# sunilsarolkarcds/ISL-SignLanguage-Translation

Hardware: AMD Instinct MI355X
Metric: frames/sec body_25 368×656 fwd+NMS+PAF at 1/8 MI355X; conv MFMA util % (higher is better)
Workload: dtype fp32 (split-fp16 x3 MFMA, fp32 accumulate)

## Files before the change

### isl-signlanguage-translation_amd/csrc/wino_f16.hip

```cpp
#include <algorithm>
#include <cstdlib>
#include <type_traits>

#include "internal.h"

namespace isl {
namespace {

typedef _Float16 f16x8 __attribute__((ext_vector_type(8)));
typedef _Float16 f16x2 __attribute__((ext_vector_type(2)));
typedef float f32x2 __attribute__((ext_vector_type(2)));
typedef float f32x4 __attribute__((ext_vector_type(4)));
typedef float f32x16 __attribute__((ext_vector_type(16)));
typedef unsigned u32x4 __attribute__((ext_vector_type(4)));

struct W2Args {
  const float* in;
  float* out;
  const f16x8* upk;
  const float* bias;
  const float* slope;
  int* range_flag;
  long long in_fs, in_chs, out_fs, out_chs;
  float wscale_inv;
  int in_pad, out_pad, H, W, TH, TW, pairs, cin_chunks, co_blocks, bpf, act, nblocks;
};

constexpr int RS = 34;
constexpr int QS = 6 * 2 * RS;
constexpr int HS = 13 * 64;
constexpr int BUF = 32 * 64;

__device__ __forceinline__ void split_dw(const f32x4& v, unsigned& h01, unsigned& h23, unsigned& l01, unsigned& l23) {
  asm("v_cvt_pk_f16_f32 %0, %1, %2" : "=v"(h01) : "v"(v.x), "v"(v.y));
  asm("v_cvt_pk_f16_f32 %0, %1, %2" : "=v"(h23) : "v"(v.z), "v"(v.w));
  asm("v_fma_mixlo_f16 %0, %1, -1.0, %2 op_sel_hi:[1,0,0]" : "=v"(l01) : "v"(h01), "v"(v.x));
  asm("v_fma_mixhi_f16 %0, %1, -1.0, %2 op_sel:[1,0,0] op_sel_hi:[1,0,0]" : "+v"(l01) : "v"(h01), "v"(v.y));
  asm("v_fma_mixlo_f16 %0, %1, -1.0, %2 op_sel_hi:[1,0,0]" : "=v"(l23) : "v"(h23), "v"(v.z));
  asm("v_fma_mixhi_f16 %0, %1, -1.0, %2 op_sel:[1,0,0] op_sel_hi:[1,0,0]" : "+v"(l23) : "v"(h23), "v"(v.w));
}

struct W2Raw {
  f32x4 aX, aY, aZ, bX, bY, bZ;
};
__device__ __forceinline__ f32x2 pk_fma_s(unsigned long long s, f32x2 b, f32x2 a) {
  f32x2 d;
  asm("v_pk_fma_f32 %0, %1, %2, %3" : "=v"(d) : "s"(s), "v"(b), "v"(a));
  return d;
}
__device__ __forceinline__ f32x2 lo2(const f32x4& v) { return f32x2{v.x, v.y}; }
__device__ __forceinline__ f32x2 hi2(const f32x4& v) { return f32x2{v.z, v.w}; }

template <int ABL, int PF>
__global__ void __launch_bounds__(512, 1) wino_f16(W2Args a) {
  __shared__ f32x4 smem[8192 + 32];

  int bid = blockIdx.x;
  {
    const int nb = a.nblocks, q = nb >> 3, r = nb & 7, xcd = bid & 7, k = bid >> 3;
    bid = (xcd < r ? xcd * (q + 1) : r * (q + 1) + (xcd - r) * q) + k;
  }
  const int co_b = bid % a.co_blocks;
  const int rest = bid / a.co_blocks;
  const int fb = rest % a.bpf;
  const int n = rest / a.bpf;

  const int tid = threadIdx.x, lane = tid & 63, h = lane >> 5, l32 = lane & 31;
  const int w = __builtin_amdgcn_readfirstlane(tid >> 6);

  if (tid < 64) {
    float* eb = (float*)(smem + 8192);
    eb[tid] = a.bias[co_b * 64 + tid];
    eb[64 + tid] = a.act == ACT_PRELU ? a.slope[co_b * 64 + tid] : 0.f;
  }

  const int BW = 2 * a.TW, s0 = fb * 64;
  const int ba = s0 / BW, bb = (s0 + 63) / BW;
  const bool two = bb > ba;
  const int txlo0 = (s0 - ba * BW) >> 1;
  const int txhi0 = two ? a.TW - 1 : (s0 + 63 - ba * BW) >> 1;
  const int w0 = 2 * (txhi0 - txlo0 + 1) + 2;
  const int w1 = two ? 2 * (((s0 + 63 - bb * BW) >> 1) + 1) + 2 : 0;
  const int Hp = a.H + 2 * a.in_pad, Wp = a.W + 2 * a.in_pad;
  const float* in_f = a.in + (size_t)n * a.in_fs;

  unsigned doff[4];
  int dch[4];
#pragma unroll
  for (int e = 0; e < 4; ++e) {
    const int p = w + 8 * e;
    const int hp = p < 26 ? p / 13 : 0;
    const int u = (p - 13 * hp) * 64 + lane;
    int t = u / RS;
    const int hc = u - t * RS;
    const int par = t & 1;
    t >>= 1;
    const int row = t % 6;
    const int qq = t / 6;
    const int v = 2 * hc + par;
    const bool s1 = v >= w0;
    const int vl = s1 ? v - w0 : v;
    const bool ok = p < 26 && qq < 2 && vl < (s1 ? w1 : w0);
    const int band = s1 ? bb : ba, txlo = s1 ? 0 : txlo0;
    const int rp = min(4 * band - 1 + row + a.in_pad, Hp - 1);
    const int cp = min(2 * txlo - 1 + vl + a.in_pad, Wp - 1);
    doff[e] = ok ? (unsigned)((rp * Wp + cp) * 8 + qq * 4) * 4u : 0u;
    dch[e] = __builtin_amdgcn_readfirstlane(hp);
  }

  const int wr = w >> 1, cpr = w & 1;
  const int ra = wr == 0 ? 0 : wr == 2 ? 2 : 1, rb = wr == 3 ? 3 : wr == 2 ? 1 : 2;
  const float sr = wr == 1 ? 1.f : -1.f, sz = cpr ? -1.f : 1.f;
  const f32x4 srv = f32x4{sr, sr, sr, sr}, szv = f32x4{sz, sz, sz, sz};
  const unsigned sru = __builtin_amdgcn_readfirstlane(__builtin_bit_cast(unsigned, sr));
  const unsigned szu = __builtin_amdgcn_readfirstlane(__builtin_bit_cast(unsigned, sz));
  const unsigned long long sr2 = (unsigned long long)sru << 32 | sru, sz2 = (unsigned long long)szu << 32 | szu;
  const unsigned lds0 = (unsigned)(__UINTPTR_TYPE__)(__attribute__((address_space(3))) void*)smem;
  const int cX = cpr ? 2 : 0, cY = cpr ? 1 : 2, cZ = cpr ? 3 : 1;
  auto toff = [&](int row, int col) { return (row * 2 + (col & 1)) * RS + (col >> 1); };
  const int to_aX = toff(ra, cX), to_aY = toff(ra, cY), to_aZ = toff(ra, cZ);
  const int to_bX = toff(rb, cX), to_bY = toff(rb, cY), to_bZ = toff(rb, cZ);
  int tb[2];
#pragma unroll
  for (int j = 0; j < 2; ++j) {
    const int s = s0 + 32 * j + l32;
    const int band = s / BW, u = s - band * BW, tx = u >> 1, typ = u & 1;
    const int hc0 = band > ba ? (w0 >> 1) + tx : tx - txlo0;
    tb[j] = h * HS + 2 * typ * 2 * RS + hc0;
  }

  const unsigned uvoff = (unsigned)lane * 16;
  auto load_a = [&](f16x8 (&A)[2][2][2], int k) __attribute__((always_inline)) {
    if constexpr ((ABL & 4) != 0) return;
    const f16x8* u0 = a.upk + ((size_t)(co_b * a.pairs + k) * 16 + 4 * wr + 2 * cpr) * 256;
    const f16x8* u1 = u0 + 256;
    asm volatile(
        "global_load_dwordx4 %0, %8, %9 offset:0\n\t"
        "global_load_dwordx4 %1, %8, %9 offset:1024\n\t"
        "global_load_dwordx4 %2, %8, %9 offset:2048\n\t"
        "global_load_dwordx4 %3, %8, %9 offset:3072\n\t"
        "global_load_dwordx4 %4, %8, %10 offset:0\n\t"
        "global_load_dwordx4 %5, %8, %10 offset:1024\n\t"
        "global_load_dwordx4 %6, %8, %10 offset:2048\n\t"
        "global_load_dwordx4 %7, %8, %10 offset:3072"
        : "=v"(A[0][0][0]), "=v"(A[0][0][1]), "=v"(A[0][1][0]), "=v"(A[0][1][1]), "=v"(A[1][0][0]),
          "=v"(A[1][0][1]), "=v"(A[1][1][0]), "=v"(A[1][1][1])
        : "v"(uvoff), "s"(u0), "s"(u1)
        : "memory");
  };
  auto dma = [&](int k, int sl) __attribute__((always_inline)) {
    if constexpr ((ABL & 8) != 0) return;
#pragma unroll
    for (int e = 0; e < 4; ++e) {
      const int ch = min(2 * k + dch[e], a.cin_chunks - 1);
      const float* src = in_f + (size_t)ch * a.in_chs;
      unsigned d = doff[e];
      asm volatile("" : "+v"(d));
      __builtin_amdgcn_global_load_lds((const void*)((const char*)src + (size_t)d),
                                       (__attribute__((address_space(3))) void*)(smem + sl * BUF + (w + 8 * e) * 64),
                                       16, 0, 0);
    }
  };

  f32x16 acc[2][2][2];
#pragma unroll
  for (int x = 0; x < 2; ++x)
#pragma unroll
    for (int i = 0; i < 2; ++i)
#pragma unroll
      for (int j = 0; j < 2; ++j)
#pragma unroll
        for (int r = 0; r < 16; ++r) acc[x][i][j][r] = 0.f;

  const unsigned oaX = lds0 + 16 * to_aX, oaY = lds0 + 16 * to_aY, oaZ = lds0 + 16 * to_aZ;
  const unsigned obX = lds0 + 16 * to_bX, obY = lds0 + 16 * to_bY, obZ = lds0 + 16 * to_bZ;
  auto rd = [&](W2Raw& r, int sl, int j, auto qc, f32x2* t) __attribute__((always_inline)) {
    constexpr int OFF = decltype(qc)::value * QS * 16;
    if constexpr ((ABL & 32) != 0) {
      asm volatile("" : "=v"(r.aX), "=v"(r.bX), "=v"(r.aY), "=v"(r.bY), "=v"(r.aZ), "=v"(r.bZ));
      return;
    }
    unsigned b = (unsigned)(tb[j] + sl * BUF) * 16;
    asm volatile("" : "+v"(b));
    const unsigned paX = b + oaX, paY = b + oaY, paZ = b + oaZ, pbX = b + obX, pbY = b + obY, pbZ = b + obZ;
#define W2_READS                           \
  "ds_read_b128 %0, %6 offset:%12\n\t"     \
  "ds_read_b128 %1, %7 offset:%12\n\t"     \
  "ds_read_b128 %2, %8 offset:%12\n\t"     \
  "ds_read_b128 %3, %9 offset:%12\n\t"     \
  "ds_read_b128 %4, %10 offset:%12\n\t"    \
  "ds_read_b128 %5, %11 offset:%12"
    if (t)
      asm volatile(W2_READS
                   : "=&v"(r.aX), "=&v"(r.bX), "=&v"(r.aY), "=&v"(r.bY), "=&v"(r.aZ), "=&v"(r.bZ)
                   : "v"(paX), "v"(pbX), "v"(paY), "v"(pbY), "v"(paZ), "v"(pbZ), "n"(OFF), "v"(t[0]), "v"(t[1]),
                     "v"(t[2]), "v"(t[3]), "v"(t[4]), "v"(t[5])
                   : "memory");
    else
      asm volatile(W2_READS
                   : "=&v"(r.aX), "=&v"(r.bX), "=&v"(r.aY), "=&v"(r.bY), "=&v"(r.aZ), "=&v"(r.bZ)
                   : "v"(paX), "v"(pbX), "v"(paY), "v"(pbY), "v"(paZ), "v"(pbZ), "n"(OFF)
                   : "memory");
#undef W2_READS
  };
  auto compute_pf = [&](const f16x8 (&A)[2][2][2], int sl, W2Raw r) __attribute__((always_inline)) {
    unsigned Bd[2][2][4];
    auto group = [&](auto jc, auto qc) __attribute__((always_inline)) {
      constexpr int j = decltype(jc)::value, Q = decltype(qc)::value;
      if constexpr ((ABL & 32) != 0) {
      } else if constexpr (j == 0 && Q == 0) {
        asm volatile("s_waitcnt lgkmcnt(0)"
                     : "+v"(r.aX), "+v"(r.bX), "+v"(r.aY), "+v"(r.bY), "+v"(r.aZ), "+v"(r.bZ)
                     :
                     : "memory");
      } else if constexpr (Q == 1) {
        asm volatile("s_waitcnt lgkmcnt(0)"
                     : "+v"(r.aX), "+v"(r.bX), "+v"(r.aY), "+v"(r.bY), "+v"(r.aZ), "+v"(r.bZ), "+v"(Bd[0][0][0]),
                       "+v"(Bd[0][0][1]), "+v"(Bd[0][1][0]), "+v"(Bd[0][1][1]), "+v"(Bd[1][0][0]), "+v"(Bd[1][0][1]),
                       "+v"(Bd[1][1][0]), "+v"(Bd[1][1][1])
                     :
                     : "memory");
      } else {
        asm volatile("s_waitcnt lgkmcnt(0)"
                     : "+v"(r.aX), "+v"(r.bX), "+v"(r.aY), "+v"(r.bY), "+v"(r.aZ), "+v"(r.bZ), "+v"(acc[0][0][0]),
                       "+v"(acc[0][1][0])
                     :
                     : "memory");
      }
      f32x2 t[6];
      t[0] = pk_fma_s(sr2, lo2(r.bX), lo2(r.aX)), t[1] = pk_fma_s(sr2, hi2(r.bX), hi2(r.aX));
      t[2] = pk_fma_s(sr2, lo2(r.bY), lo2(r.aY)), t[3] = pk_fma_s(sr2, hi2(r.bY), hi2(r.aY));
      t[4] = pk_fma_s(sr2, lo2(r.bZ), lo2(r.aZ)), t[5] = pk_fma_s(sr2, hi2(r.bZ), hi2(r.aZ));
      if constexpr (Q == 0) rd(r, sl, j, std::integral_constant<int, 1>{}, t);
      else if constexpr (j == 0) rd(r, sl, 1, std::integral_constant<int, 0>{}, t);
      if constexpr (j == 0 || Q == 0) __builtin_amdgcn_sched_barrier(0);
      const f32x2 v00 = t[0] - t[2], v01 = t[1] - t[3];
      const f32x2 v10 = pk_fma_s(sz2, t[4], t[2]), v11 = pk_fma_s(sz2, t[5], t[3]);
      split_dw(f32x4{v00.x, v00.y, v01.x, v01.y}, Bd[0][0][2 * Q], Bd[0][0][2 * Q + 1], Bd[0][1][2 * Q], Bd[0][1][2 * Q + 1]);
      split_dw(f32x4{v10.x, v10.y, v11.x, v11.y}, Bd[1][0][2 * Q], Bd[1][0][2 * Q + 1], Bd[1][1][2 * Q], Bd[1][1][2 * Q + 1]);
      if constexpr (Q == 1) {
        f16x8 Bh[2], Bl[2];
#pragma unroll
        for (int x = 0; x < 2; ++x) {
          Bh[x] = __builtin_bit_cast(f16x8, u32x4{Bd[x][0][0], Bd[x][0][1], Bd[x][0][2], Bd[x][0][3]});
          Bl[x] = __builtin_bit_cast(f16x8, u32x4{Bd[x][1][0], Bd[x][1][1], Bd[x][1][2], Bd[x][1][3]});
        }
#pragma unroll
        for (int x = 0; x < 2; ++x)
#pragma unroll
          for (int i = 0; i < 2; ++i) {
            if constexpr ((ABL & 1) != 0) continue;
            acc[x][i][j] = __builtin_amdgcn_mfma_f32_32x32x16_f16(A[x][i][0], Bh[x], acc[x][i][j], 0, 0, 0);
            acc[x][i][j] = __builtin_amdgcn_mfma_f32_32x32x16_f16(A[x][i][0], Bl[x], acc[x][i][j], 0, 0, 0);
            acc[x][i][j] = __builtin_amdgcn_mfma_f32_32x32x16_f16(A[x][i][1], Bh[x], acc[x][i][j], 0, 0, 0);
          }
      }
    };
    group(std::integral_constant<int, 0>{}, std::integral_constant<int, 0>{});
    group(std::integral_constant<int, 0>{}, std::integral_constant<int, 1>{});
    group(std::integral_constant<int, 1>{}, std::integral_constant<int, 0>{});
    group(std::integral_constant<int, 1>{}, std::integral_constant<int, 1>{});
  };

  auto compute = [&](const f16x8 (&A)[2][2][2], int sl) __attribute__((always_inline)) {
#pragma unroll
    for (int j = 0; j < 2; ++j) {
      int b = tb[j] + sl * BUF;
      asm volatile("" : "+v"(b));
      unsigned Bd[2][2][4];
      if constexpr ((ABL & 2) != 0) {
#pragma unroll
        for (int x = 0; x < 2; ++x)
#pragma unroll
          for (int hl = 0; hl < 2; ++hl)
#pragma unroll
            for (int d = 0; d < 4; ++d) Bd[x][hl][d] = 0x3c003c00u;
      } else {
        auto quad = [&](auto qc) __attribute__((always_inline)) {
          constexpr int Q = decltype(qc)::value;
          const f32x4 aX = smem[b + to_aX + Q * QS], aY = smem[b + to_aY + Q * QS], aZ = smem[b + to_aZ + Q * QS];
          const f32x4 bX = smem[b + to_bX + Q * QS], bY = smem[b + to_bY + Q * QS], bZ = smem[b + to_bZ + Q * QS];
          const f32x4 tX = __builtin_elementwise_fma(srv, bX, aX);
          const f32x4 tY = __builtin_elementwise_fma(srv, bY, aY);
          const f32x4 tZ = __builtin_elementwise_fma(srv, bZ, aZ);
          const f32x4 v0 = tX - tY;
          const f32x4 v1 = __builtin_elementwise_fma(szv, tZ, tY);
          split_dw(v0, Bd[0][0][2 * Q], Bd[0][0][2 * Q + 1], Bd[0][1][2 * Q], Bd[0][1][2 * Q + 1]);
          split_dw(v1, Bd[1][0][2 * Q], Bd[1][0][2 * Q + 1], Bd[1][1][2 * Q], Bd[1][1][2 * Q + 1]);
        };
        quad(std::integral_constant<int, 0>{});
        quad(std::integral_constant<int, 1>{});
      }
      f16x8 Bh[2], Bl[2];
#pragma unroll
      for (int x = 0; x < 2; ++x) {
        Bh[x] = __builtin_bit_cast(f16x8, u32x4{Bd[x][0][0], Bd[x][0][1], Bd[x][0][2], Bd[x][0][3]});
        Bl[x] = __builtin_bit_cast(f16x8, u32x4{Bd[x][1][0], Bd[x][1][1], Bd[x][1][2], Bd[x][1][3]});
      }
#pragma unroll
      for (int x = 0; x < 2; ++x)
#pragma unroll
        for (int i = 0; i < 2; ++i) {
          if constexpr ((ABL & 1) != 0) continue;
          acc[x][i][j] = __builtin_amdgcn_mfma_f32_32x32x16_f16(A[x][i][0], Bh[x], acc[x][i][j], 0, 0, 0);
          acc[x][i][j] = __builtin_amdgcn_mfma_f32_32x32x16_f16(A[x][i][0], Bl[x], acc[x][i][j], 0, 0, 0);
          acc[x][i][j] = __builtin_amdgcn_mfma_f32_32x32x16_f16(A[x][i][1], Bh[x], acc[x][i][j], 0, 0, 0);
        }
    }
  };

  f16x8 AS[2][2][2][2];
  load_a(AS[0], 0);
  dma(0, 0);
  dma(min(1, a.pairs - 1), 1);
  asm volatile("s_waitcnt vmcnt(4)" ::: "memory");
  __syncthreads();
  __builtin_amdgcn_sched_barrier(0);
  auto step = [&](int k, f16x8 (&A)[2][2][2], f16x8 (&An)[2][2][2]) __attribute__((always_inline)) {
    W2Raw r0;
    if constexpr (PF != 0) rd(r0, k % 3, 0, std::integral_constant<int, 0>{}, nullptr);
    load_a(An, min(k + 1, a.pairs - 1));
    dma(min(k + 2, a.pairs - 1), (k + 2) % 3);
    __builtin_amdgcn_sched_barrier(0);
    if constexpr ((ABL & 4) == 0)
      asm volatile("s_waitcnt vmcnt(16)"
                   : "+v"(A[0][0][0]), "+v"(A[0][0][1]), "+v"(A[0][1][0]), "+v"(A[0][1][1]), "+v"(A[1][0][0]),
                     "+v"(A[1][0][1]), "+v"(A[1][1][0]), "+v"(A[1][1][1])
                   :
                   : "memory");
    if constexpr (PF != 0) compute_pf(A, k % 3, r0);
    else compute(A, k % 3);
    __builtin_amdgcn_sched_barrier(0);
    asm volatile("s_waitcnt vmcnt(12) lgkmcnt(0)" ::: "memory");
    __builtin_amdgcn_s_barrier();
    __builtin_amdgcn_sched_barrier(0);
  };
  for (int k = 0; k < a.pairs; k += 2) {
    step(k, AS[0], AS[1]);
    if (k + 1 < a.pairs) step(k + 1, AS[1], AS[0]);
  }
  asm volatile("s_waitcnt vmcnt(0) lgkmcnt(0)"
               : "+v"(AS[0][0][0][0]), "+v"(AS[0][0][0][1]), "+v"(AS[0][0][1][0]), "+v"(AS[0][0][1][1]),
                 "+v"(AS[0][1][0][0]), "+v"(AS[0][1][0][1]), "+v"(AS[0][1][1][0]), "+v"(AS[0][1][1][1]),
                 "+v"(AS[1][0][0][0]), "+v"(AS[1][0][0][1]), "+v"(AS[1][0][1][0]), "+v"(AS[1][0][1][1]),
                 "+v"(AS[1][1][0][0]), "+v"(AS[1][1][0][1]), "+v"(AS[1][1][1][0]), "+v"(AS[1][1][1][1])
               :
               : "memory");
  __syncthreads();

  bool bad = false;
  if constexpr ((ABL & 16) != 0) {
    float sum = 0.f;
#pragma unroll
    for (int x = 0; x < 2; ++x)
#pragma unroll
      for (int i = 0; i < 2; ++i)
#pragma unroll
        for (int j = 0; j < 2; ++j)
#pragma unroll
          for (int r = 0; r < 16; ++r) sum += acc[x][i][j][r];
    if (sum == 1.2345f || bad) atomicOr(a.range_flag, 1);
    return;
  }
  f32x4* xm = smem;
  const float* eb = (const float*)(smem + 8192);
  const int Wo = a.W + 2 * a.out_pad;
  float* out_f = a.out + (size_t)n * a.out_fs;
  const int rn = tid & 31, rh = (tid >> 5) & 1, rq = (tid >> 6) & 3, rj = tid >> 8;
  const int rs = s0 + 32 * rj + rn, rband = rs / BW, ru = rs - rband * BW, rtx = ru >> 1, rty = 2 * rband + (ru & 1);
#pragma unroll
  for (int i = 0; i < 2; ++i) {
#pragma unroll
    for (int x = 0; x < 2; ++x)
#pragma unroll
      for (int j = 0; j < 2; ++j)
#pragma unroll
        for (int q = 0; q < 4; ++q)
          xm[((((2 * w + x) * 2 + j) * 4 + q) * 2 + h) * 32 + l32] =
              f32x4{acc[x][i][j][4 * q], acc[x][i][j][4 * q + 1], acc[x][i][j][4 * q + 2], acc[x][i][j][4 * q + 3]};
    __syncthreads();
    {
      const f32x4* mp = xm + ((rj * 4 + rq) * 2 + rh) * 32 + rn;
      f32x4 R0[4], R1[4];
#pragma unroll
      for (int c = 0; c < 4; ++c) {
        const f32x4 m0 = mp[(0 + c) * 512], m1 = mp[(4 + c) * 512], m2 = mp[(8 + c) * 512], m3 = mp[(12 + c) * 512];
        R0[c] = (m0 + m1) + m2;
        R1[c] = (m1 - m2) - m3;
      }
      f32x4 Y[2][2];
      Y[0][0] = (R0[0] + R0[1]) + R0[2];
      Y[0][1] = (R0[1] - R0[2]) - R0[3];
      Y[1][0] = (R1[0] + R1[1]) + R1[2];
      Y[1][1] = (R1[1] - R1[2]) - R1[3];
      const int cl = i * 32 + 8 * rq + 4 * rh, co = co_b * 64 + cl;
      const f32x4 bv = *(const f32x4*)(eb + cl);
      const f32x4 sl = *(const f32x4*)(eb + 64 + cl);
      if (rty < a.TH) {
        float* oc = out_f + (size_t)(co >> 3) * a.out_chs + (co & 7);
#pragma unroll
        for (int yy = 0; yy < 2; ++yy)
#pragma unroll
          for (int xx = 0; xx < 2; ++xx) {
            const int y = 2 * rty + yy, x = 2 * rtx + xx;
            if (y >= a.H || x >= a.W) continue;
            f32x4 v;
#pragma unroll
            for (int e = 0; e < 4; ++e) v[e] = Y[yy][xx][e] * a.wscale_inv + bv[e];
            if (a.act == ACT_RELU) {
#pragma unroll
              for (int e = 0; e < 4; ++e) v[e] = v[e] > 0.f ? v[e] : 0.f;
            } else if (a.act == ACT_PRELU) {
#pragma unroll
              for (int e = 0; e < 4; ++e) v[e] = v[e] >= 0.f ? v[e] : v[e] * sl[e];
            }
#pragma unroll
            for (int e = 0; e < 4; ++e) bad |= !(__builtin_fabsf(v[e]) < 65504.f);
            *(f32x4*)(oc + (size_t)((y + a.out_pad) * Wo + x + a.out_pad) * 8) = v;
          }
      }
    }
    __syncthreads();
  }
  if (bad) atomicOr(a.range_flag, 1);
}

int g_wino_blocks(const ConvLaunch& c, int* bpf) {
  const int TH = (c.H + 1) / 2, TW = (c.W + 1) / 2, nbands = (TH + 1) / 2;
  *bpf = (nbands * 2 * TW + 63) / 64;
  return c.n * *bpf * (c.cout / 64);
}

}

bool wino_f16_fits(const ConvLaunch& c) {
  return c.ks == 3 && c.in_pad >= 1 && c.cout % 64 == 0 && c.cout > 0 && !c.hpool && !c.vin && !c.fold &&
         c.cout7 == 0 && (c.W + 1) / 2 >= 32 && (long long)c.H * c.W > 1024 &&
         !((c.in_cs | c.in_coff | c.out_cs | c.out_coff) & 7) && (long long)(c.H + 2 * c.in_pad) * (c.W + 2 * c.in_pad) * 8 < (1ll << 30);
}

hipError_t launch_wino_f16(const ConvLaunch& c, hipStream_t s) {
  if (!wino_f16_fits(c)) { set_error("wino_f16: launch not eligible"); return hipErrorInvalidValue; }
  if (!c.wx3 || !c.range_flag) { set_error("wino_f16: split filters / range flag missing"); return hipErrorInvalidValue; }
  W2Args a{};
  a.in_chs = (long long)(c.H + 2 * c.in_pad) * (c.W + 2 * c.in_pad) * 8;
  a.out_chs = (long long)(c.H + 2 * c.out_pad) * (c.W + 2 * c.out_pad) * 8;
  a.in_fs = a.in_chs * (c.in_cs / 8);
  a.out_fs = a.out_chs * (c.out_cs / 8);
  a.in = c.in + (c.in_coff / 8) * a.in_chs;
  a.out = c.out + (c.out_coff / 8) * a.out_chs;
  a.upk = (const f16x8*)c.wx3;
  a.bias = c.bias;
  a.slope = c.slope;
  a.range_flag = c.range_flag;
  a.wscale_inv = c.wscale_inv;
  a.in_pad = c.in_pad;
  a.out_pad = c.out_pad;
  a.H = c.H;
  a.W = c.W;
  a.TH = (c.H + 1) / 2;
  a.TW = (c.W + 1) / 2;
  a.pairs = (c.cin_chunks + 1) / 2;
  a.cin_chunks = c.cin_chunks;
  a.co_blocks = c.cout / 64;
  a.act = c.act;
  const long long nb = g_wino_blocks(c, &a.bpf);
  if (nb <= 0 || nb > 0x7fffffff) { set_error("wino_f16: bad grid"); return hipErrorInvalidValue; }
  a.nblocks = (int)nb;
#ifdef ISLPOSE_DEV
  const int abl = getenv("ISLPOSE_W2_ABL") ? atoi(getenv("ISLPOSE_W2_ABL")) : 0;
  switch (abl) {
#define W2ABL(k) case k: hipLaunchKernelGGL((wino_f16<k, 0>), dim3(a.nblocks), dim3(512), 0, s, a); return hipGetLastError();
    W2ABL(1) W2ABL(2) W2ABL(3) W2ABL(4) W2ABL(6) W2ABL(8) W2ABL(12) W2ABL(14) W2ABL(16) W2ABL(31)
#undef W2ABL
    case 65: hipLaunchKernelGGL((wino_f16<1, 1>), dim3(a.nblocks), dim3(512), 0, s, a); return hipGetLastError();
    case 68: hipLaunchKernelGGL((wino_f16<4, 1>), dim3(a.nblocks), dim3(512), 0, s, a); return hipGetLastError();
    case 72: hipLaunchKernelGGL((wino_f16<8, 1>), dim3(a.nblocks), dim3(512), 0, s, a); return hipGetLastError();
    case 76: hipLaunchKernelGGL((wino_f16<12, 1>), dim3(a.nblocks), dim3(512), 0, s, a); return hipGetLastError();
    case 80: hipLaunchKernelGGL((wino_f16<16, 1>), dim3(a.nblocks), dim3(512), 0, s, a); return hipGetLastError();
    case 32: hipLaunchKernelGGL((wino_f16<32, 1>), dim3(a.nblocks), dim3(512), 0, s, a); return hipGetLastError();
    default: break;
  }
  if (getenv("ISLPOSE_W2_PF") && atoi(getenv("ISLPOSE_W2_PF")) == 0) {
    hipLaunchKernelGGL((wino_f16<0, 0>), dim3(a.nblocks), dim3(512), 0, s, a);
    return hipGetLastError();
  }
#endif
  hipLaunchKernelGGL((wino_f16<0, 1>), dim3(a.nblocks), dim3(512), 0, s, a);
  return hipGetLastError();
}

double wino_f16_mfma_flops(const ConvLaunch& c) {
  int bpf = 0;
  const double nb = g_wino_blocks(c, &bpf);
  return nb * 16.0 * 64 * 64 * 16.0 * ((c.cin_chunks + 1) / 2) * 2 * 3;
}

}
```

Before: 1372.

## Interleave input DMA with B-transform and use scalar-operand transform asm

```diff
diff --git a/isl-signlanguage-translation_amd/csrc/wino_f16.hip b/isl-signlanguage-translation_amd/csrc/wino_f16.hip
--- a/isl-signlanguage-translation_amd/csrc/wino_f16.hip
+++ b/isl-signlanguage-translation_amd/csrc/wino_f16.hip
@@ -43,6 +43,60 @@
 struct W2Raw {
   f32x4 aX, aY, aZ, bX, bY, bZ;
 };
+__device__ __forceinline__ void rows_s(unsigned s, f32x4& tX, f32x4& tY, f32x4& tZ, const W2Raw& r) {
+  asm("v_fma_f32 %0, %36, %24, %12\n\t"
+      "v_fma_f32 %1, %36, %25, %13\n\t"
+      "v_fma_f32 %2, %36, %26, %14\n\t"
+      "v_fma_f32 %3, %36, %27, %15\n\t"
+      "v_fma_f32 %4, %36, %28, %16\n\t"
+      "v_fma_f32 %5, %36, %29, %17\n\t"
+      "v_fma_f32 %6, %36, %30, %18\n\t"
+      "v_fma_f32 %7, %36, %31, %19\n\t"
+      "v_fma_f32 %8, %36, %32, %20\n\t"
+      "v_fma_f32 %9, %36, %33, %21\n\t"
+      "v_fma_f32 %10, %36, %34, %22\n\t"
+      "v_fma_f32 %11, %36, %35, %23"
+      : "=&v"(tX.x), "=&v"(tX.y), "=&v"(tX.z), "=&v"(tX.w), "=&v"(tY.x), "=&v"(tY.y), "=&v"(tY.z), "=&v"(tY.w),
+        "=&v"(tZ.x), "=&v"(tZ.y), "=&v"(tZ.z), "=&v"(tZ.w)
+      : "v"(r.aX.x), "v"(r.aX.y), "v"(r.aX.z), "v"(r.aX.w), "v"(r.aY.x), "v"(r.aY.y), "v"(r.aY.z), "v"(r.aY.w),
+        "v"(r.aZ.x), "v"(r.aZ.y), "v"(r.aZ.z), "v"(r.aZ.w), "v"(r.bX.x), "v"(r.bX.y), "v"(r.bX.z), "v"(r.bX.w),
+        "v"(r.bY.x), "v"(r.bY.y), "v"(r.bY.z), "v"(r.bY.w), "v"(r.bZ.x), "v"(r.bZ.y), "v"(r.bZ.z), "v"(r.bZ.w), "s"(s));
+}
+__device__ __forceinline__ void cols_s(unsigned sz, f32x4& tX, const f32x4& tY, f32x4& tZ) {
+  asm("v_sub_f32 %0, %0, %8\n\t"
+      "v_sub_f32 %1, %1, %9\n\t"
+      "v_sub_f32 %2, %2, %10\n\t"
+      "v_sub_f32 %3, %3, %11\n\t"
+      "v_fma_f32 %4, %12, %4, %8\n\t"
+      "v_fma_f32 %5, %12, %5, %9\n\t"
+      "v_fma_f32 %6, %12, %6, %10\n\t"
+      "v_fma_f32 %7, %12, %7, %11"
+      : "+v"(tX.x), "+v"(tX.y), "+v"(tX.z), "+v"(tX.w), "+v"(tZ.x), "+v"(tZ.y), "+v"(tZ.z), "+v"(tZ.w)
+      : "v"(tY.x), "v"(tY.y), "v"(tY.z), "v"(tY.w), "s"(sz));
+}
+template <bool mfma_next>
+__device__ __forceinline__ void split_dw2(const f32x4& v0, const f32x4& v1, unsigned& h0a, unsigned& h0b, unsigned& l0a,
+                                          unsigned& l0b, unsigned& h1a, unsigned& h1b, unsigned& l1a, unsigned& l1b) {
+#define W2_SPLIT2(tail)                                                          \
+  asm("v_cvt_pk_f16_f32 %0, %8, %9\n\t"                                          \
+      "v_cvt_pk_f16_f32 %1, %10, %11\n\t"                                        \
+      "v_cvt_pk_f16_f32 %4, %12, %13\n\t"                                        \
+      "v_cvt_pk_f16_f32 %5, %14, %15\n\t"                                        \
+      "v_fma_mixlo_f16 %2, %0, -1.0, %8 op_sel_hi:[1,0,0]\n\t"                   \
+      "v_fma_mixlo_f16 %3, %1, -1.0, %10 op_sel_hi:[1,0,0]\n\t"                  \
+      "v_fma_mixlo_f16 %6, %4, -1.0, %12 op_sel_hi:[1,0,0]\n\t"                  \
+      "v_fma_mixlo_f16 %7, %5, -1.0, %14 op_sel_hi:[1,0,0]\n\t"                  \
+      "v_fma_mixhi_f16 %2, %0, -1.0, %9 op_sel:[1,0,0] op_sel_hi:[1,0,0]\n\t"    \
+      "v_fma_mixhi_f16 %3, %1, -1.0, %11 op_sel:[1,0,0] op_sel_hi:[1,0,0]\n\t"   \
+      "v_fma_mixhi_f16 %6, %4, -1.0, %13 op_sel:[1,0,0] op_sel_hi:[1,0,0]\n\t"   \
+      "v_fma_mixhi_f16 %7, %5, -1.0, %15 op_sel:[1,0,0] op_sel_hi:[1,0,0]" tail    \
+      : "=&v"(h0a), "=&v"(h0b), "=&v"(l0a), "=&v"(l0b), "=&v"(h1a), "=&v"(h1b), "=&v"(l1a), "=&v"(l1b) \
+      : "v"(v0.x), "v"(v0.y), "v"(v0.z), "v"(v0.w), "v"(v1.x), "v"(v1.y), "v"(v1.z), "v"(v1.w))
+  if constexpr (mfma_next) W2_SPLIT2("\n\ts_nop 1");
+  else W2_SPLIT2("");
+#undef W2_SPLIT2
+}
+#ifdef ISLPOSE_DEV
 __device__ __forceinline__ f32x2 pk_fma_s(unsigned long long s, f32x2 b, f32x2 a) {
   f32x2 d;
   asm("v_pk_fma_f32 %0, %1, %2, %3" : "=v"(d) : "s"(s), "v"(b), "v"(a));
@@ -50,8 +104,9 @@
 }
 __device__ __forceinline__ f32x2 lo2(const f32x4& v) { return f32x2{v.x, v.y}; }
 __device__ __forceinline__ f32x2 hi2(const f32x4& v) { return f32x2{v.z, v.w}; }
-
-template <int ABL, int PF>
+#endif
+
+template <int ABL, int SC>
 __global__ void __launch_bounds__(512, 1) wino_f16(W2Args a) {
   __shared__ f32x4 smem[8192 + 32];
 
@@ -111,7 +166,6 @@
   const int wr = w >> 1, cpr = w & 1;
   const int ra = wr == 0 ? 0 : wr == 2 ? 2 : 1, rb = wr == 3 ? 3 : wr == 2 ? 1 : 2;
   const float sr = wr == 1 ? 1.f : -1.f, sz = cpr ? -1.f : 1.f;
-  const f32x4 srv = f32x4{sr, sr, sr, sr}, szv = f32x4{sz, sz, sz, sz};
   const unsigned sru = __builtin_amdgcn_readfirstlane(__builtin_bit_cast(unsigned, sr));
   const unsigned szu = __builtin_amdgcn_readfirstlane(__builtin_bit_cast(unsigned, sz));
   const unsigned long long sr2 = (unsigned long long)sru << 32 | sru, sz2 = (unsigned long long)szu << 32 | szu;
@@ -148,18 +202,19 @@
         : "v"(uvoff), "s"(u0), "s"(u1)
         : "memory");
   };
+  auto dma_piece = [&](int k, int sl, int e) __attribute__((always_inline)) {
+    if constexpr ((ABL & 8) != 0) return;
+    const int ch = min(2 * k + dch[e], a.cin_chunks - 1);
+    const float* src = in_f + (size_t)ch * a.in_chs;
+    unsigned d = doff[e];
+    asm volatile("" : "+v"(d));
+    __builtin_amdgcn_global_load_lds((const void*)((const char*)src + (size_t)d),
+                                     (__attribute__((address_space(3))) void*)(smem + sl * BUF + (w + 8 * e) * 64),
+                                     16, 0, 0);
+  };
   auto dma = [&](int k, int sl) __attribute__((always_inline)) {
-    if constexpr ((ABL & 8) != 0) return;
-#pragma unroll
-    for (int e = 0; e < 4; ++e) {
-      const int ch = min(2 * k + dch[e], a.cin_chunks - 1);
-      const float* src = in_f + (size_t)ch * a.in_chs;
-      unsigned d = doff[e];
-      asm volatile("" : "+v"(d));
-      __builtin_amdgcn_global_load_lds((const void*)((const char*)src + (size_t)d),
-                                       (__attribute__((address_space(3))) void*)(smem + sl * BUF + (w + 8 * e) * 64),
-                                       16, 0, 0);
-    }
+#pragma unroll
+    for (int e = 0; e < 4; ++e) dma_piece(k, sl, e);
   };
 
   f32x16 acc[2][2][2];
@@ -174,7 +229,7 @@
 
   const unsigned oaX = lds0 + 16 * to_aX, oaY = lds0 + 16 * to_aY, oaZ = lds0 + 16 * to_aZ;
   const unsigned obX = lds0 + 16 * to_bX, obY = lds0 + 16 * to_bY, obZ = lds0 + 16 * to_bZ;
-  auto rd = [&](W2Raw& r, int sl, int j, auto qc, f32x2* t) __attribute__((always_inline)) {
+  auto rd = [&](W2Raw& r, int sl, int j, auto qc, auto* t) __attribute__((always_inline)) {
     constexpr int OFF = decltype(qc)::value * QS * 16;
     if constexpr ((ABL & 32) != 0) {
       asm volatile("" : "=v"(r.aX), "=v"(r.bX), "=v"(r.aY), "=v"(r.bY), "=v"(r.aZ), "=v"(r.bZ));
@@ -190,20 +245,25 @@
   "ds_read_b128 %3, %9 offset:%12\n\t"     \
   "ds_read_b128 %4, %10 offset:%12\n\t"    \
   "ds_read_b128 %5, %11 offset:%12"
-    if (t)
+    if constexpr (std::is_same_v<decltype(t), std::nullptr_t*>)
+      asm volatile(W2_READS
+                   : "=&v"(r.aX), "=&v"(r.bX), "=&v"(r.aY), "=&v"(r.bY), "=&v"(r.aZ), "=&v"(r.bZ)
+                   : "v"(paX), "v"(pbX), "v"(paY), "v"(pbY), "v"(paZ), "v"(pbZ), "n"(OFF)
+                   : "memory");
+    else if constexpr (std::is_same_v<decltype(t), f32x4*>)
+      asm volatile(W2_READS
+                   : "=&v"(r.aX), "=&v"(r.bX), "=&v"(r.aY), "=&v"(r.bY), "=&v"(r.aZ), "=&v"(r.bZ)
+                   : "v"(paX), "v"(pbX), "v"(paY), "v"(pbY), "v"(paZ), "v"(pbZ), "n"(OFF), "v"(t[0].x)
+                   : "memory");
+    else
       asm volatile(W2_READS
                    : "=&v"(r.aX), "=&v"(r.bX), "=&v"(r.aY), "=&v"(r.bY), "=&v"(r.aZ), "=&v"(r.bZ)
                    : "v"(paX), "v"(pbX), "v"(paY), "v"(pbY), "v"(paZ), "v"(pbZ), "n"(OFF), "v"(t[0]), "v"(t[1]),
                      "v"(t[2]), "v"(t[3]), "v"(t[4]), "v"(t[5])
                    : "memory");
-    else
-      asm volatile(W2_READS
-                   : "=&v"(r.aX), "=&v"(r.bX), "=&v"(r.aY), "=&v"(r.bY), "=&v"(r.aZ), "=&v"(r.bZ)
-                   : "v"(paX), "v"(pbX), "v"(paY), "v"(pbY), "v"(paZ), "v"(pbZ), "n"(OFF)
-                   : "memory");
 #undef W2_READS
   };
-  auto compute_pf = [&](const f16x8 (&A)[2][2][2], int sl, W2Raw r) __attribute__((always_inline)) {
+  auto compute = [&](const f16x8 (&A)[2][2][2], int sl, W2Raw r, int kd, int sld) __attribute__((always_inline)) {
     unsigned Bd[2][2][4];
     auto group = [&](auto jc, auto qc) __attribute__((always_inline)) {
       constexpr int j = decltype(jc)::value, Q = decltype(qc)::value;
@@ -227,17 +287,36 @@
                      :
                      : "memory");
       }
-      f32x2 t[6];
-      t[0] = pk_fma_s(sr2, lo2(r.bX), lo2(r.aX)), t[1] = pk_fma_s(sr2, hi2(r.bX), hi2(r.aX));
-      t[2] = pk_fma_s(sr2, lo2(r.bY), lo2(r.aY)), t[3] = pk_fma_s(sr2, hi2(r.bY), hi2(r.aY));
-      t[4] = pk_fma_s(sr2, lo2(r.bZ), lo2(r.aZ)), t[5] = pk_fma_s(sr2, hi2(r.bZ), hi2(r.aZ));
-      if constexpr (Q == 0) rd(r, sl, j, std::integral_constant<int, 1>{}, t);
-      else if constexpr (j == 0) rd(r, sl, 1, std::integral_constant<int, 0>{}, t);
-      if constexpr (j == 0 || Q == 0) __builtin_amdgcn_sched_barrier(0);
-      const f32x2 v00 = t[0] - t[2], v01 = t[1] - t[3];
-      const f32x2 v10 = pk_fma_s(sz2, t[4], t[2]), v11 = pk_fma_s(sz2, t[5], t[3]);
-      split_dw(f32x4{v00.x, v00.y, v01.x, v01.y}, Bd[0][0][2 * Q], Bd[0][0][2 * Q + 1], Bd[0][1][2 * Q], Bd[0][1][2 * Q + 1]);
-      split_dw(f32x4{v10.x, v10.y, v11.x, v11.y}, Bd[1][0][2 * Q], Bd[1][0][2 * Q + 1], Bd[1][1][2 * Q], Bd[1][1][2 * Q + 1]);
+      auto next_reads = [&](auto* t) __attribute__((always_inline)) {
+        if constexpr (Q == 0) rd(r, sl, j, std::integral_constant<int, 1>{}, t);
+        else if constexpr (j == 0) rd(r, sl, 1, std::integral_constant<int, 0>{}, t);
+        if constexpr (j == 0 || Q == 0) __builtin_amdgcn_sched_barrier(0);
+      };
+      if constexpr (SC != 0) {
+        f32x4 t[3];
+        rows_s(sru, t[0], t[1], t[2], r);
+        next_reads(t);
+        cols_s(szu, t[0], t[1], t[2]);
+        split_dw2<Q == 1>(t[0], t[2], Bd[0][0][2 * Q], Bd[0][0][2 * Q + 1], Bd[0][1][2 * Q], Bd[0][1][2 * Q + 1],
+                          Bd[1][0][2 * Q], Bd[1][0][2 * Q + 1], Bd[1][1][2 * Q], Bd[1][1][2 * Q + 1]);
+      }
+#ifdef ISLPOSE_DEV
+      else {
+        f32x2 t[6];
+        t[0] = pk_fma_s(sr2, lo2(r.bX), lo2(r.aX)), t[1] = pk_fma_s(sr2, hi2(r.bX), hi2(r.aX));
+        t[2] = pk_fma_s(sr2, lo2(r.bY), lo2(r.aY)), t[3] = pk_fma_s(sr2, hi2(r.bY), hi2(r.aY));
+        t[4] = pk_fma_s(sr2, lo2(r.bZ), lo2(r.aZ)), t[5] = pk_fma_s(sr2, hi2(r.bZ), hi2(r.aZ));
+        next_reads(t);
+        const f32x2 v00 = t[0] - t[2], v01 = t[1] - t[3];
+        const f32x2 v10 = pk_fma_s(sz2, t[4], t[2]), v11 = pk_fma_s(sz2, t[5], t[3]);
+        split_dw(f32x4{v00.x, v00.y, v01.x, v01.y}, Bd[0][0][2 * Q], Bd[0][0][2 * Q + 1], Bd[0][1][2 * Q], Bd[0][1][2 * Q + 1]);
+        split_dw(f32x4{v10.x, v10.y, v11.x, v11.y}, Bd[1][0][2 * Q], Bd[1][0][2 * Q + 1], Bd[1][1][2 * Q], Bd[1][1][2 * Q + 1]);
+      }
+#endif
+      if constexpr (SC != 0) {
+        dma_piece(kd, sld, 2 * j + Q);
+        __builtin_amdgcn_sched_barrier(0);
+      }
       if constexpr (Q == 1) {
         f16x8 Bh[2], Bl[2];
 #pragma unroll
@@ -260,53 +339,6 @@
     group(std::integral_constant<int, 0>{}, std::integral_constant<int, 1>{});
     group(std::integral_constant<int, 1>{}, std::integral_constant<int, 0>{});
     group(std::integral_constant<int, 1>{}, std::integral_constant<int, 1>{});
-  };
-
-  auto compute = [&](const f16x8 (&A)[2][2][2], int sl) __attribute__((always_inline)) {
-#pragma unroll
-    for (int j = 0; j < 2; ++j) {
-      int b = tb[j] + sl * BUF;
-      asm volatile("" : "+v"(b));
-      unsigned Bd[2][2][4];
-      if constexpr ((ABL & 2) != 0) {
-#pragma unroll
-        for (int x = 0; x < 2; ++x)
-#pragma unroll
-          for (int hl = 0; hl < 2; ++hl)
-#pragma unroll
-            for (int d = 0; d < 4; ++d) Bd[x][hl][d] = 0x3c003c00u;
-      } else {
-        auto quad = [&](auto qc) __attribute__((always_inline)) {
-          constexpr int Q = decltype(qc)::value;
-          const f32x4 aX = smem[b + to_aX + Q * QS], aY = smem[b + to_aY + Q * QS], aZ = smem[b + to_aZ + Q * QS];
-          const f32x4 bX = smem[b + to_bX + Q * QS], bY = smem[b + to_bY + Q * QS], bZ = smem[b + to_bZ + Q * QS];
-          const f32x4 tX = __builtin_elementwise_fma(srv, bX, aX);
-          const f32x4 tY = __builtin_elementwise_fma(srv, bY, aY);
-          const f32x4 tZ = __builtin_elementwise_fma(srv, bZ, aZ);
-          const f32x4 v0 = tX - tY;
-          const f32x4 v1 = __builtin_elementwise_fma(szv, tZ, tY);
-          split_dw(v0, Bd[0][0][2 * Q], Bd[0][0][2 * Q + 1], Bd[0][1][2 * Q], Bd[0][1][2 * Q + 1]);
-          split_dw(v1, Bd[1][0][2 * Q], Bd[1][0][2 * Q + 1], Bd[1][1][2 * Q], Bd[1][1][2 * Q + 1]);
-        };
-        quad(std::integral_constant<int, 0>{});
-        quad(std::integral_constant<int, 1>{});
-      }
-      f16x8 Bh[2], Bl[2];
-#pragma unroll
-      for (int x = 0; x < 2; ++x) {
-        Bh[x] = __builtin_bit_cast(f16x8, u32x4{Bd[x][0][0], Bd[x][0][1], Bd[x][0][2], Bd[x][0][3]});
-        Bl[x] = __builtin_bit_cast(f16x8, u32x4{Bd[x][1][0], Bd[x][1][1], Bd[x][1][2], Bd[x][1][3]});
-      }
-#pragma unroll
-      for (int x = 0; x < 2; ++x)
-#pragma unroll
-        for (int i = 0; i < 2; ++i) {
-          if constexpr ((ABL & 1) != 0) continue;
-          acc[x][i][j] = __builtin_amdgcn_mfma_f32_32x32x16_f16(A[x][i][0], Bh[x], acc[x][i][j], 0, 0, 0);
-          acc[x][i][j] = __builtin_amdgcn_mfma_f32_32x32x16_f16(A[x][i][0], Bl[x], acc[x][i][j], 0, 0, 0);
-          acc[x][i][j] = __builtin_amdgcn_mfma_f32_32x32x16_f16(A[x][i][1], Bh[x], acc[x][i][j], 0, 0, 0);
-        }
-    }
   };
 
   f16x8 AS[2][2][2][2];
@@ -318,18 +350,17 @@
   __builtin_amdgcn_sched_barrier(0);
   auto step = [&](int k, f16x8 (&A)[2][2][2], f16x8 (&An)[2][2][2]) __attribute__((always_inline)) {
     W2Raw r0;
-    if constexpr (PF != 0) rd(r0, k % 3, 0, std::integral_constant<int, 0>{}, nullptr);
+    rd(r0, k % 3, 0, std::integral_constant<int, 0>{}, (std::nullptr_t*)nullptr);
     load_a(An, min(k + 1, a.pairs - 1));
-    dma(min(k + 2, a.pairs - 1), (k + 2) % 3);
+    if constexpr (SC == 0) dma(min(k + 2, a.pairs - 1), (k + 2) % 3);
     __builtin_amdgcn_sched_barrier(0);
     if constexpr ((ABL & 4) == 0)
-      asm volatile("s_waitcnt vmcnt(16)"
+      asm volatile("s_waitcnt vmcnt(%8)"
                    : "+v"(A[0][0][0]), "+v"(A[0][0][1]), "+v"(A[0][1][0]), "+v"(A[0][1][1]), "+v"(A[1][0][0]),
                      "+v"(A[1][0][1]), "+v"(A[1][1][0]), "+v"(A[1][1][1])
-                   :
+                   : "n"(SC != 0 ? 12 : 16)
                    : "memory");
-    if constexpr (PF != 0) compute_pf(A, k % 3, r0);
-    else compute(A, k % 3);
+    compute(A, k % 3, r0, min(k + 2, a.pairs - 1), (k + 2) % 3);
     __builtin_amdgcn_sched_barrier(0);
     asm volatile("s_waitcnt vmcnt(12) lgkmcnt(0)" ::: "memory");
     __builtin_amdgcn_s_barrier();
@@ -469,21 +500,15 @@
   a.nblocks = (int)nb;
 #ifdef ISLPOSE_DEV
   const int abl = getenv("ISLPOSE_W2_ABL") ? atoi(getenv("ISLPOSE_W2_ABL")) : 0;
-  switch (abl) {
-#define W2ABL(k) case k: hipLaunchKernelGGL((wino_f16<k, 0>), dim3(a.nblocks), dim3(512), 0, s, a); return hipGetLastError();
-    W2ABL(1) W2ABL(2) W2ABL(3) W2ABL(4) W2ABL(6) W2ABL(8) W2ABL(12) W2ABL(14) W2ABL(16) W2ABL(31)
+  const int sc = getenv("ISLPOSE_W2_SC") ? atoi(getenv("ISLPOSE_W2_SC")) : 1;
+  switch (sc * 100 + abl) {
+#define W2VAR(c, k) case c * 100 + k: hipLaunchKernelGGL((wino_f16<k, c>), dim3(a.nblocks), dim3(512), 0, s, a); return hipGetLastError();
+#define W2ABL(c) W2VAR(c, 1) W2VAR(c, 4) W2VAR(c, 8) W2VAR(c, 12) W2VAR(c, 16) W2VAR(c, 32)
+    W2VAR(0, 0) W2ABL(0) W2ABL(1)
 #undef W2ABL
-    case 65: hipLaunchKernelGGL((wino_f16<1, 1>), dim3(a.nblocks), dim3(512), 0, s, a); return hipGetLastError();
-    case 68: hipLaunchKernelGGL((wino_f16<4, 1>), dim3(a.nblocks), dim3(512), 0, s, a); return hipGetLastError();
-    case 72: hipLaunchKernelGGL((wino_f16<8, 1>), dim3(a.nblocks), dim3(512), 0, s, a); return hipGetLastError();
-    case 76: hipLaunchKernelGGL((wino_f16<12, 1>), dim3(a.nblocks), dim3(512), 0, s, a); return hipGetLastError();
-    case 80: hipLaunchKernelGGL((wino_f16<16, 1>), dim3(a.nblocks), dim3(512), 0, s, a); return hipGetLastError();
-    case 32: hipLaunchKernelGGL((wino_f16<32, 1>), dim3(a.nblocks), dim3(512), 0, s, a); return hipGetLastError();
-    default: break;
-  }
-  if (getenv("ISLPOSE_W2_PF") && atoi(getenv("ISLPOSE_W2_PF")) == 0) {
-    hipLaunchKernelGGL((wino_f16<0, 0>), dim3(a.nblocks), dim3(512), 0, s, a);
-    return hipGetLastError();
+#undef W2VAR
+    case 100: break;
+    default: set_error("wino_f16: no such development variant"); return hipErrorInvalidValue;
   }
 #endif
   hipLaunchKernelGGL((wino_f16<0, 1>), dim3(a.nblocks), dim3(512), 0, s, a);
```

New measurement: 1378, median of 6. About the same (+0.5%).
